# jiahuei/COMIC-Compact-Image-Captioning-with-Attention

Hardware: AMD Instinct MI355X
Metric: images/sec (decoder-mode XE training, COMIC-256, InceptionV3 frozen) (higher is better)
Workload: dtype bf16

## Files before the change

### comic-compact-image-captioning-with-attention_amd/_lib.py

```python
import ctypes as C
import os

_HERE = os.path.dirname(os.path.abspath(__file__))
LIB_PATH = os.environ.get('COMIC_HIP_LIB') or os.path.join(_HERE, 'lib', 'libcomic_hip.so')

c_void_p, c_int, c_int32, c_int64, c_float, c_double, c_char_p, c_uint64 = (
    C.c_void_p, C.c_int, C.c_int32, C.c_int64, C.c_float, C.c_double, C.c_char_p, C.c_uint64)


class CnnOp(C.Structure):
    _fields_ = [(n, c_int32) for n in (
        'kind', 'src', 'dst', 'src_coff', 'dst_coff', 'H', 'W', 'Cin', 'Cout', 'KH', 'KW', 'SH', 'SW',
        'PT', 'PL', 'Ho', 'Wo', 'weight', 'relu', 'out_f32', 'src_f32', 'lane', 'tile', 'group', 'flags', 'min_lds')]


class ImageDesc(C.Structure):
    _fields_ = [('offset', C.c_int64), ('in_h', c_int32), ('in_w', c_int32), ('flip', c_int32), ('oy', c_int32),
                ('ox', c_int32), ('sy', C.c_float), ('sx', C.c_float)]


class ConvWeight(C.Structure):
    _fields_ = [('w', c_void_p), ('scale', c_void_p), ('shift', c_void_p), ('w_frag', c_void_p)]


# ... 23 lines not shown
_DEC_ENV = (('COMIC_PERSIST', '0', DEC_NO_PERSIST), ('COMIC_PERSIST_BWD', '0', DEC_NO_PERSIST_BWD),
            ('COMIC_FUSED_STEP', '0', DEC_NO_FUSED_STEP), ('COMIC_SPLIT_ATTN_BWD', '0', DEC_NO_SPLIT_ATTN_BWD),
            ('COMIC_GRAD_LANES', '0', DEC_ONE_LANE), ('COMIC_SPLIT3', '0', DEC_EXACT_GEMM),
            ('COMIC_PERSIST_STAMPS', '1', DEC_STAMPS), ('COMIC_BEAM_LOGITS', '0', DEC_NO_BEAM_LOGITS),
            ('COMIC_LSTM_STREAM', '0', DEC_NO_LSTM_STREAM), ('COMIC_GROUP_GEMM', '0', DEC_NO_GROUP_GEMM),
            ('COMIC_BWD_OWN_ROWS', '1', DEC_BWD_OWN_ROWS))


def decoder_flags_from_env():
    f = 0
    for name, val, bit in _DEC_ENV:
        if os.environ.get(name, '')[:1] == val:
            f |= bit
    return f


CONV_TILES = 61
WS_TILE = 54
IMG_TILE = 55
CHAIN_TILE = 62
OP_RAW, OP_POOLED_SRC, OP_X3 = 1, 2, 4
OP_CHAIN_LINK = 8
OP_CHAIN_KEEP = 16
IM2COL_CONV_TILES = 12


def is_im2col_tile(tile):
    return tile <= IM2COL_CONV_TILES or 26 <= tile <= 47
PARAM_NAMES = ('W_init', 'K', 'b', 'W_m', 'W_v', 'W_q', 'v', 'ln_g', 'ln_b', 'tau', 'W_a', 'W_o', 'b_o', 'emb', 'cell_ln', 'K_c', 'b_c', 'status')


class DecoderParams(C.Structure):
    _fields_ = [(n, c_void_p) for n in PARAM_NAMES]


class BeamConstraints(C.Structure):
    _fields_ = [(n, c_int32) for n in ('min_length', 'no_repeat_ngram', 'ngram_stride', 'n_suppress')] + [
        ('suppress', c_int32 * 32)]


class GemmProb(C.Structure):
    _fields_ = [(n, c_void_p) for n in ('A', 'B', 'C', 'bias', 'mask')] + [(n, c_int32) for n in (
        'M', 'N', 'K', 'lda', 'ldb', 'ldc', 'ld_mask')] + [(n, c_float) for n in ('alpha', 'beta', 'keep')] + [
        ('type', c_int32), ('ones_a', c_int32)]


# ... 200 lines not shown
```

### comic-compact-image-captioning-with-attention_amd/csrc/conv.hip

```cpp
#include "conv_common.h"
#include "conv_ws.h"
#include "conv_stem.h"
#include "conv_img.h"
#include <cstdlib>
#include <cstring>
#include <algorithm>
#include <vector>

namespace {

constexpr int kRowBytes = 80;

template <typename T, int BM, int BN, int WM, int WN, bool MASK = false>
__global__ __launch_bounds__(256) void conv_igemm_kernel(ConvArgs a) {
  constexpr int EPC = Elem<T>::EPC;
  constexpr int BKE = 4 * EPC;
  constexpr int A_PASSES = (BM + 63) / 64;
  constexpr int B_PASSES = (BN + 63) / 64;
  constexpr int TM = BM / WM / 16;
  constexpr int TN = BN / WN / 16;
  static_assert(WM * WN == 4, "4 waves");

  __shared__ __attribute__((aligned(16))) unsigned char smem[2 * (BM + BN) * kRowBytes];
  unsigned char* Xs = smem;
// ... 2198 lines not shown
  while (j < n_ops && ops[j].group == ops[i].group) ++j;
  return j - i;
}

}

extern "C" long comic_cnn_group_args_bytes(const comic_cnn_op* ops, int n_ops) {
  long n = 0;
  for (int i = 0; i < n_ops; ++i) n += ops[i].group > 0;
  return n * (long)sizeof(ConvArgs);
}

extern "C" int comic_cnn_build_group_args(const comic_cnn_op* ops, int n_ops, void* const* buffers,
                                          const int32_t* buf_channels, const comic_conv_weight* weights, int batch,
                                          void* host_out) {
  COMIC_REQUIRE(ops && buffers && buf_channels && weights && host_out, "comic_cnn_build_group_args: null argument");
  ConvArgs* out = (ConvArgs*)host_out;
  for (int i = 0; i < n_ops;) {
    const int n = group_run(ops, n_ops, i);
    if (ops[i].group <= 0) {
      ++i;
      continue;
    }
    if (ws_group_selected(ops + i, n, batch)) {
      memset(out, 0, sizeof(ConvArgs) * n);
      out += n;
      i += n;
      continue;
    }
    COMIC_REQUIRE(ops[i].tile != COMIC_WS_TILE, "conv: group is not eligible for the weight-stationary 1x1 kernel");
    const int tile = group_tile(ops + i, n, batch);
    for (int j = 0; j < n; ++j)
      COMIC_REQUIRE(tile == COMIC_CHAIN_TILE || !(ops[i + j].flags & COMIC_OP_CHAIN_LINK),
                    "conv: COMIC_OP_CHAIN_LINK ops depend on each other -- their group runs on COMIC_CHAIN_TILE only (got tile %d)", tile);
    if (tile == COMIC_IMG_TILE || tile == COMIC_CHAIN_TILE) {
      memset(out, 0, sizeof(ConvArgs) * n);
      out += n;
      i += n;
      continue;
    }
    int blk = 0;
    for (int j = 0; j < n; ++j) {
      const comic_cnn_op* op = ops + i + j;
      const comic_conv_weight* wt = weights + op->weight;
      if (int rc = validate_grouped_conv(op, buf_channels[op->src], buf_channels[op->dst], wt, batch)) return rc;
      COMIC_REQUIRE(buffers[op->src] && buffers[op->dst], "grouped conv: null buffer");
      ConvArgs& a = out[j];
// ... 55 lines not shown
}

namespace {
struct Lanes {
  hipStream_t s[3];
  hipEvent_t fork_ev, join_ev[3];
  bool ok = false;
};
Lanes* get_lanes() {
  static Lanes lanes[16];
  int dev = 0;
  if (hipGetDevice(&dev) != hipSuccess || dev < 0 || dev >= 16) return nullptr;
  Lanes& l = lanes[dev];
  if (!l.ok) {
    for (int i = 0; i < 3; ++i) {
      if (hipStreamCreateWithFlags(&l.s[i], hipStreamNonBlocking) != hipSuccess) return nullptr;
      if (hipEventCreateWithFlags(&l.join_ev[i], hipEventDisableTiming) != hipSuccess) return nullptr;
    }
    if (hipEventCreateWithFlags(&l.fork_ev, hipEventDisableTiming) != hipSuccess) return nullptr;
    l.ok = true;
  }
  return &l;
}
}

template <typename HT>
static int cnn_forward_impl(const comic_cnn_op* ops, int n_ops, void* const* buffers, const int32_t* buf_channels,
                            const comic_conv_weight* weights, int batch, int dtype, const void* group_args_dev,
                            void* stream) {
  COMIC_REQUIRE(ops && buffers && buf_channels, "comic_cnn_forward: null table");
  const ConvArgs* gargs = (const ConvArgs*)group_args_dev;
  hipStream_t main_st = (hipStream_t)stream;
  Lanes* lanes = nullptr;
  bool used[3] = {false, false, false};
  for (int i = 0; i < n_ops; ++i) {
    const comic_cnn_op* op = ops + i;
    if (op->kind == 5) {
      if (!lanes) lanes = get_lanes();
      COMIC_REQUIRE(lanes, "comic_cnn_forward: cannot create branch streams");
      COMIC_REQUIRE(hipEventRecord(lanes->fork_ev, main_st) == hipSuccess, "fork: event record failed");
      for (int l = 0; l < 3; ++l) {
        COMIC_REQUIRE(hipStreamWaitEvent(lanes->s[l], lanes->fork_ev, 0) == hipSuccess, "fork: wait failed");
        used[l] = false;
      }
      continue;
    }
    if (op->kind == 6) {
      COMIC_REQUIRE(lanes, "join without fork");
      for (int l = 0; l < 3; ++l) {
        if (!used[l]) continue;
        COMIC_REQUIRE(hipEventRecord(lanes->join_ev[l], lanes->s[l]) == hipSuccess, "join: event record failed");
        COMIC_REQUIRE(hipStreamWaitEvent(main_st, lanes->join_ev[l], 0) == hipSuccess, "join: wait failed");
      }
      continue;
    }
    if (gargs && op->group > 0) {
      COMIC_REQUIRE(dtype == Half16<HT>::code && (op->kind == 0 || op->kind == 7) && op->lane == 0,
                    "grouped launch needs a bf16 or f16 plan and conv / pool+bn ops on the caller's stream");
      const int n = group_run(ops, n_ops, i);
      if (ws_group_selected(op, n, batch)) {
        if (int rc = run_ws_group<HT>(op, n, buffers, buf_channels, weights, batch, main_st)) return rc;
        gargs += n;
        i += n - 1;
        continue;
      }
      COMIC_REQUIRE(op->tile != COMIC_WS_TILE, "conv: group is not eligible for the weight-stationary 1x1 kernel");
      const int tile = group_tile(op, n, batch);
      for (int j = 0; j < n; ++j)
        COMIC_REQUIRE(tile == COMIC_CHAIN_TILE || !(op[j].flags & COMIC_OP_CHAIN_LINK),
                      "conv: COMIC_OP_CHAIN_LINK ops depend on each other -- their group runs on COMIC_CHAIN_TILE only (got tile %d)", tile);
      if (tile == COMIC_CHAIN_TILE) {
        if (int rc = launch_img_chains<HT>(op, n, buffers, buf_channels, weights, batch, main_st)) return rc;
        COMIC_LAUNCH_CHECK("image-resident conv chains");
        gargs += n;
        i += n - 1;
        continue;
      }
      if (tile == COMIC_IMG_TILE) {
// ... 32 lines not shown
        int lds = 0;
        const long nb = member_blocks(tile, a, &lds);
        COMIC_REQUIRE(nb >= 0, "grouped launch: member %d is not eligible for patch tile %d", j, tile);
        blocks += nb;
        lds_max = std::max(lds_max, lds);
      }
      COMIC_REQUIRE(blocks > 0 && blocks < (1L << 31), "grouped launch: bad workgroup count");
      if (is_walk_tile(tile)) blocks = (long)cdiv(batch * op->Ho * op->Wo, tile_bm(tile)) * walk_split(tile);
      if (!is_im2col_tile(tile)) {
        if (int rc = launch_patch_grouped_tile<HT>(tile, gargs, n, (int)blocks, std::max(lds_max, op->min_lds), main_st)) return rc;
      } else if (int rc = launch_dma_grouped_tile<HT>(tile, gargs, n, (int)blocks, op->min_lds, main_st)) {
        return rc;
      }
      COMIC_LAUNCH_CHECK("grouped conv");
      gargs += n;
      i += n - 1;
      continue;
    }
    hipStream_t st = main_st;
    if (op->lane > 0) {
      COMIC_REQUIRE(lanes && op->lane <= 3, "branch lane %d outside a fork/join region", op->lane);
      st = lanes->s[op->lane - 1];
      used[op->lane - 1] = true;
    }
    if (op->kind == 8 || op->kind == 9) {
      const bool with_1a = op->kind == 9;
      const int H0 = with_1a ? (op->H - 3) / 2 + 1 : op->H, W0 = with_1a ? (op->W - 3) / 2 + 1 : op->W;
      COMIC_REQUIRE(dtype == Half16<HT>::code && op->lane == 0, "stem stream: bf16 / f16 plans on the caller's stream only");
      COMIC_REQUIRE(op->Cin == (with_1a ? 3 : 32) && op->Cout == 64 && op->KH == 3 && op->KW == 3 && op->SH == 1 && op->SW == 1,
                    "stem stream: expects the (3 ->) 32 -> 32 -> 64 3x3 stem (got Cin %d, Cout %d)", op->Cin, op->Cout);
      COMIC_REQUIRE(comic_stem_stream_supported(H0, W0) && (!with_1a || comic_stem_stream_1a_supported(op->H, op->W)),
                    "stem stream: map %dx%d is not supported", op->H, op->W);
      const int Hp = (H0 - 2 - 3) / 2 + 1, Wp = (W0 - 2 - 3) / 2 + 1;
      COMIC_REQUIRE(op->Ho == Hp && op->Wo == Wp, "stem stream: Ho/Wo must be the pooled grid %dx%d", Hp, Wp);
      const comic_conv_weight* w0 = with_1a ? weights + op->weight : nullptr;
      const comic_conv_weight* wa = weights + op->weight + (with_1a ? 1 : 0);
      const comic_conv_weight* wb = wa + 1;
      const int xc = buf_channels[op->src], yc = buf_channels[op->dst];
      COMIC_REQUIRE(buffers[op->src] && buffers[op->dst] && wa->w && wb->w && wa->scale && wa->shift && wb->scale && wb->shift,
                    "stem stream: null buffer / weights");
      COMIC_REQUIRE(op->dst_coff + 64 <= yc && yc % 4 == 0 && op->dst_coff % 4 == 0, "stem stream: bad destination slice");
      COMIC_REQUIRE((long)batch * Hp * Wp * yc * 2 < (1L << 31), "stem stream: tensor too large");
      ComicStemArgs sa{};
      if (with_1a) {
        COMIC_REQUIRE(w0->w && w0->scale && w0->shift && xc == 3 && op->src_coff == 0, "stem stream: Conv2d_1a needs the whole fp32 image");
        sa.img = (const float*)buffers[op->src]; sa.Hi = op->H; sa.Wi = op->W;
        sa.w0 = (const float*)w0->w; sa.sc0 = w0->scale; sa.sh0 = w0->shift;
        sa.x = nullptr; sa.x_cs = 32; sa.x_co = 0;
      } else {
        COMIC_REQUIRE(op->src_coff + 32 <= xc && xc % 8 == 0 && op->src_coff % 8 == 0, "stem stream: bad source slice");
        COMIC_REQUIRE((long)batch * op->H * op->W * xc * 2 < (1L << 31), "stem stream: tensor too large");
        sa.x = (const bf16_t*)buffers[op->src]; sa.x_cs = xc; sa.x_co = op->src_coff;
      }
      sa.B = batch; sa.H0 = H0; sa.W0 = W0;
      sa.w1 = (const bf16_t*)wa->w; sa.w2 = (const bf16_t*)wb->w; sa.Kpad = (9 * 32 + 63) / 64 * 64;
      sa.sc1 = wa->scale; sa.sh1 = wa->shift; sa.sc2 = wb->scale; sa.sh2 = wb->shift;
      sa.y = (bf16_t*)buffers[op->dst]; sa.y_cs = yc; sa.y_co = op->dst_coff; sa.Hp = Hp; sa.Wp = Wp;
      sa.n_tasks = 2 * batch;
      sa.f16 = std::is_same<HT, f16_t>::value;
      if (int rc = comic_stem_stream_launch(sa, main_st)) return rc;
      COMIC_LAUNCH_CHECK("stem stream");
      continue;
    }
    const comic_conv_weight* wt = (op->kind <= 1 || op->kind == 7) ? weights + op->weight : nullptr;
    int rc = comic_conv2d_bn_relu(op, buffers[op->src], buf_channels[op->src], buffers[op->dst],
                                  buf_channels[op->dst], wt, batch, dtype, (void*)st);
    if (rc) return rc;
  }
  return 0;
}

extern "C" int comic_cnn_forward(const comic_cnn_op* ops, int n_ops, void* const* buffers, const int32_t* buf_channels,
                                 const comic_conv_weight* weights, int batch, int dtype, void* stream) {
  if (dtype == COMIC_F16) return cnn_forward_impl<f16_t>(ops, n_ops, buffers, buf_channels, weights, batch, dtype, nullptr, stream);
  return cnn_forward_impl<bf16_t>(ops, n_ops, buffers, buf_channels, weights, batch, dtype, nullptr, stream);
}

extern "C" int comic_cnn_forward_grouped(const comic_cnn_op* ops, int n_ops, void* const* buffers,
                                         const int32_t* buf_channels, const comic_conv_weight* weights, int batch,
                                         int dtype, const void* group_args_dev, void* stream) {
  COMIC_REQUIRE(group_args_dev || comic_cnn_group_args_bytes(ops, n_ops) == 0,
                "comic_cnn_forward_grouped: plan has grouped ops but no argument records");
  if (dtype == COMIC_F16)
    return cnn_forward_impl<f16_t>(ops, n_ops, buffers, buf_channels, weights, batch, dtype, group_args_dev, stream);
  return cnn_forward_impl<bf16_t>(ops, n_ops, buffers, buf_channels, weights, batch, dtype, group_args_dev, stream);
// ... 1484 lines not shown
```

### comic-compact-image-captioning-with-attention_amd/csrc/conv_stem.h

```cpp
#pragma once
#include "conv_common.h"

struct ComicStemArgs {
  const bf16_t* x;
  int B, H0, W0, x_cs, x_co;
  const bf16_t* w1;
  const bf16_t* w2;
  int Kpad;
  const float *sc1, *sh1, *sc2, *sh2;
  bf16_t* y;
  int y_cs, y_co, Hp, Wp;
  int n_tasks, parts;
  const float* img;
  int Hi, Wi;
  const float* w0;
  const float *sc0, *sh0;
  int f16;
};

bool comic_stem_stream_supported(int H0, int W0);
bool comic_stem_stream_1a_supported(int Hi, int Wi);
int comic_stem_stream_launch(const ComicStemArgs& a, hipStream_t st);
```

### comic-compact-image-captioning-with-attention_amd/csrc/conv_stem.hip

```cpp
#include <algorithm>

#include "conv_common.h"
#include "conv_stem.h"

namespace {

constexpr int kPxB = 96;
constexpr int kRowPx = 132;
constexpr int kRowB = kRowPx * kPxB;
constexpr int kRing = 4;
constexpr int kTableFloats = 2 * (32 + 64);
constexpr int kImgRing = 16;

#define STEM_BARRIER()                                    \
  do {                                                    \
    asm volatile("s_waitcnt lgkmcnt(0)" ::: "memory");    \
    __builtin_amdgcn_s_barrier();                         \
    asm volatile("" ::: "memory");                        \
  } while (0)

__device__ __forceinline__ float row_next1(float v) { return dpp_move<0x12F>(v, v); }
__device__ __forceinline__ float row_next2(float v) { return dpp_move<0x12E>(v, v); }

template <typename HT, bool FUSE1A>
__global__ __launch_bounds__(512) void conv_stem_stream_kernel(ComicStemArgs a) {
  extern __shared__ __attribute__((aligned(16))) unsigned char smem[];
  float* table = (float*)smem;
  unsigned char* xring = smem + kTableFloats * 4;
  unsigned char* yring = xring + kRing * kRowB;
  float* imgring = (float*)(yring + kRing * kRowB);

  const int tid = threadIdx.x, lane = tid & 63;
  const int wave = __builtin_amdgcn_readfirstlane(tid >> 6);
  const int H1 = a.H0 - 2, W1 = a.W0 - 2;
  const int part_rows = (a.Hp + a.parts - 1) / a.parts;

  if (tid < 32) {
    table[tid] = a.sc1[tid];
    table[32 + tid] = a.sh1[tid];
  }
  if (tid < 64) {
    table[64 + tid] = a.sc2[tid];
    table[128 + tid] = a.sh2[tid];
  }
  for (int i = tid; i < kRing * kRowPx * (kPxB / 16); i += 512) *(uint4*)(yring + i * 16) = make_uint4(0, 0, 0, 0);
  if constexpr (FUSE1A)
    for (int i = tid; i < kImgRing * a.Wi * 3 / 4; i += 512) *(float4*)(imgring + 4 * i) = make_float4(0.f, 0.f, 0.f, 0.f);

  const int fr = lane & 15, fg = lane >> 4;
  const uint32_t x_lane = (uint32_t)(fr * kPxB + fg * 16);

  if (wave >= 4) {
    const int wv = wave - 4;
    const int p = wv & 1, hh = wv >> 1;
    const int y1_start = 64 * hh;
    const bool y1_work = y1_start < W1;
    const int ltid = tid - 256;
    int px[2], ch[2];
    bool act[2];
#pragma unroll
    for (int i = 0; i < 2; ++i) {
      const int c = ltid + 256 * i;
      px[i] = c >> 2;
      ch[i] = c & 3;
      act[i] = px[i] < a.W0;
    }
    uint32_t goff[2];
#pragma unroll
// ... 82 lines not shown
        const int x = 32 * wv + 16 * i + fr;
        const int x6 = 6 * min(x, a.W0 - 1);
        float xv[8];
#pragma unroll
        for (int s8 = 0; s8 < 8; ++s8) xv[s8] = imgring[rb[s8] + x6];
        uint32_t hh[4], ll[4];
#pragma unroll
        for (int e = 0; e < 4; ++e) {
          hh[e] = pack_bf16x2(xv[2 * e], xv[2 * e + 1]);
          ll[e] = pack_bf16x2(xv[2 * e] - __uint_as_float(hh[e] << 16), xv[2 * e + 1] - __uint_as_float(hh[e] & 0xFFFF0000u));
        }
        const bf16x8_t xh = __builtin_bit_cast(bf16x8_t, make_uint4(hh[0], hh[1], hh[2], hh[3]));
        const bf16x8_t xl = __builtin_bit_cast(bf16x8_t, make_uint4(ll[0], ll[1], ll[2], ll[3]));
#pragma unroll
        for (int n = 0; n < 2; ++n) {
          f32x4_t acc0 = (f32x4_t){0.f, 0.f, 0.f, 0.f};
          acc0 = __builtin_amdgcn_mfma_f32_16x16x32_bf16(w0h[n], xh, acc0, 0, 0, 0);
          acc0 = __builtin_amdgcn_mfma_f32_16x16x32_bf16(w0h[n], xl, acc0, 0, 0, 0);
          acc0 = __builtin_amdgcn_mfma_f32_16x16x32_bf16(w0l[n], xh, acc0, 0, 0, 0);
          const float v0 = fmaxf(fmaf(acc0[0], sc0[n].x, sh0[n].x), 0.f), v1 = fmaxf(fmaf(acc0[1], sc0[n].y, sh0[n].y), 0.f);
          const float v2 = fmaxf(fmaf(acc0[2], sc0[n].z, sh0[n].z), 0.f), v3 = fmaxf(fmaf(acc0[3], sc0[n].w, sh0[n].w), 0.f);
          if (x < a.W0) *(uint2*)(dst + x * kPxB + n * 32) = make_uint2(Half16<HT>::pack(v0, v1), Half16<HT>::pack(v2, v3));
        }
      }
    };
    STEM_BARRIER();
    const float4 sc1 = *(const float4*)(table + p * 16 + fg * 4), sh1 = *(const float4*)(table + 32 + p * 16 + fg * 4);
    for (int task = blockIdx.x; task < a.n_tasks; task += gridDim.x) {
      const int b = task / a.parts, h = task - b * a.parts;
      const int p0 = h * part_rows, p1 = min(a.Hp, p0 + part_rows) - 1;
      const int qa = 2 * p0 - 1, r_last = 2 * p1 + 2;
      const int nsteps = r_last + 2 - qa + 1;
      Row r0, r1, r2;
      ImgRows ia, ib, ic;
      if constexpr (FUSE1A) {
        const int ir0 = 2 * max(qa, 0), ir1 = min(2 * (qa + 3) + 2, a.Hi - 1);
        const float4* src = (const float4*)(a.img + ((size_t)b * a.Hi + ir0) * rowf);
        for (int i = ltid; i < (ir1 - ir0 + 1) * row4; i += 256) {
          const int r = ir0 + i / row4, c4 = i % row4;
          *(float4*)(imgring + (size_t)(r & (kImgRing - 1)) * rowf + 4 * c4) = src[i];
        }
        ia = load_img(b, qa + 4);
        ib = load_img(b, qa + 5);
        STEM_BARRIER();
        compute_x0(qa);
        compute_x0(qa + 1);
// ... 37 lines not shown
            }
            __builtin_amdgcn_s_setprio(0);
          }
          unsigned char* dst = yring + ((q + 8) & 3) * kRowB + (p * 16 + fg * 4) * 2;
#pragma unroll
          for (int j = 0; j < 4; ++j) {
            const int x = y1_start + j * 16 + fr;
            float v0 = fmaxf(fmaf(acc[j][0], sc1.x, sh1.x), 0.f), v1 = fmaxf(fmaf(acc[j][1], sc1.y, sh1.y), 0.f);
            float v2 = fmaxf(fmaf(acc[j][2], sc1.z, sh1.z), 0.f), v3 = fmaxf(fmaf(acc[j][3], sc1.w, sh1.w), 0.f);
            if (!real) v0 = v1 = v2 = v3 = 0.f;
            if (x < W1) *(uint2*)(dst + (x + 1) * kPxB) = make_uint2(Half16<HT>::pack(v0, v1), Half16<HT>::pack(v2, v3));
          }
        }
        if constexpr (FUSE1A) {
          compute_x0(q + 3);
          store_img(q + 4, ia);
          ia = ib;
          ib = ic;
        } else {
          store_row(q + 3, r0);
          r0 = r1;
          r1 = r2;
        }
        STEM_BARRIER();
      }
    }
    return;
  }

  const int p = wave & 1, hh = wave >> 1;
  const int y2_start = 56 * hh;
  const bool y2_work = y2_start < W1;
  constexpr int kTileStep = 14;
  bf16x8_t w2[2][9];
#pragma unroll
  for (int i = 0; i < 2; ++i) {
    const bf16_t* wp2 = a.w2 + (size_t)((2 * p + i) * 16 + fr) * a.Kpad + fg * 8;
#pragma unroll
    for (int tap = 0; tap < 9; ++tap) w2[i][tap] = __builtin_bit_cast(bf16x8_t, *(const uint4*)(wp2 + tap * 32));
  }
  STEM_BARRIER();
  float4 sc2[2], sh2[2];
#pragma unroll
  for (int i = 0; i < 2; ++i) {
    sc2[i] = *(const float4*)(table + 64 + (2 * p + i) * 16 + fg * 4);
    sh2[i] = *(const float4*)(table + 128 + (2 * p + i) * 16 + fg * 4);
  }

// ... 48 lines not shown
      const int prow = p0 + (rel >> 1) - 1;
#pragma unroll
      for (int i = 0; i < 2; ++i) {
        f32x4_t v[4];
#pragma unroll
        for (int j = 0; j < 4; ++j)
#pragma unroll
          for (int e = 0; e < 4; ++e) {
            v[j][e] = fmaxf(run[i][j][e], acc[i][j][e]);
            run[i][j][e] = acc[i][j][e];
          }
#pragma unroll
        for (int j = 0; j < 4; ++j) {
          float o[4];
#pragma unroll
          for (int e = 0; e < 4; ++e)
            o[e] = fmaxf(fmaxf(v[j][e], row_next1(v[j][e])), row_next2(v[j][e]));
          const float o0 = fmaxf(fmaf(o[0], sc2[i].x, sh2[i].x), 0.f), o1 = fmaxf(fmaf(o[1], sc2[i].y, sh2[i].y), 0.f);
          const float o2 = fmaxf(fmaf(o[2], sc2[i].z, sh2[i].z), 0.f), o3 = fmaxf(fmaf(o[3], sc2[i].w, sh2[i].w), 0.f);
          const int x = y2_start + j * kTileStep + fr;
          const int jc = x >> 1;
          if ((fr & 1) == 0 && fr <= 12 && jc < a.Wp) {
            bf16_t* yp = a.y + ((size_t)((b * a.Hp + prow) * a.Wp + jc)) * a.y_cs + a.y_co + (2 * p + i) * 16 + fg * 4;
            *(uint2*)yp = make_uint2(Half16<HT>::pack(o0, o1), Half16<HT>::pack(o2, o3));
          }
        }
      }
    };
    f32x4_t acc[2][4];
    for (int t = 0; t < nsteps; ++t) {
      const int r = qa + t - 2;
      if (y2_work && r >= r_first && r <= r_last) {
        mfma_row(r, acc);
        pool_row(r, acc);
      }
      STEM_BARRIER();
    }
  }
}

}

bool comic_stem_stream_supported(int H0, int W0) {
  const int Wp = (W0 - 2 - 3) / 2 + 1;
  return H0 >= 7 && W0 >= 7 && Wp <= 56;
}

bool comic_stem_stream_1a_supported(int Hi, int Wi) {
  const int H0 = (Hi - 3) / 2 + 1, W0 = (Wi - 3) / 2 + 1;
  return Hi >= 17 && Wi % 4 == 0 && 2 * (Wi * 3 / 4) <= 512 && comic_stem_stream_supported(H0, W0) &&
         kTableFloats * 4 + 2 * kRing * kRowB + kImgRing * Wi * 3 * 4 <= 160 * 1024;
}

namespace {
template <typename HT>
int stem_stream_launch(const ComicStemArgs& a_in, hipStream_t st) {
  ComicStemArgs a = a_in;
  if (!comic_stem_stream_supported(a.H0, a.W0) || (a.img && !comic_stem_stream_1a_supported(a.Hi, a.Wi))) {
    comic_set_error("conv_stem: unsupported map %dx%d", a.H0, a.W0);
    return 2;
  }
  const int lds = kTableFloats * 4 + 2 * kRing * kRowB + (a.img ? kImgRing * a.Wi * 3 * 4 : 0);
  static PerDeviceOnce attr_once__;
  bool& attr_set = attr_once__.slot();
  if (!attr_set) {
    if (hipFuncSetAttribute((const void*)conv_stem_stream_kernel<HT, false>, hipFuncAttributeMaxDynamicSharedMemorySize,
                            160 * 1024) != hipSuccess ||
        hipFuncSetAttribute((const void*)conv_stem_stream_kernel<HT, true>, hipFuncAttributeMaxDynamicSharedMemorySize,
                            160 * 1024) != hipSuccess) {
      comic_set_error("conv_stem: cannot reserve %d bytes of LDS", lds);
      return 1;
    }
    attr_set = true;
  }
  int dev = 0, cus = 256;
  if (hipGetDevice(&dev) == hipSuccess) (void)hipDeviceGetAttribute(&cus, hipDeviceAttributeMultiprocessorCount, dev);
  a.parts = 2;
  while (a.parts < 8 && a.B * a.parts < cus && (a.Hp + 2 * a.parts - 1) / (2 * a.parts) >= 6) a.parts *= 2;
  a.n_tasks = a.B * a.parts;
  const int grid = std::min(a.n_tasks, cus);
  if (a.img)
    hipLaunchKernelGGL((conv_stem_stream_kernel<HT, true>), dim3(grid), dim3(512), lds, st, a);
  else
    hipLaunchKernelGGL((conv_stem_stream_kernel<HT, false>), dim3(grid), dim3(512), lds, st, a);
  return 0;
}
}

int comic_stem_stream_launch(const ComicStemArgs& a, hipStream_t st) {
  return a.f16 ? stem_stream_launch<f16_t>(a, st) : stem_stream_launch<bf16_t>(a, st);
}
```

### comic-compact-image-captioning-with-attention_amd/nets.py

```python
from __future__ import annotations

import ctypes as C
import json
import math
import os

import numpy as np

from . import _lib as L
from . import streams

BN_EPS = 1e-3

_STEM = [('c', 'Conv2d_1a_3x3', 32, (3, 3), 2, 'VALID'), ('c', 'Conv2d_2a_3x3', 32, (3, 3), 1, 'VALID'),
         ('c', 'Conv2d_2b_3x3', 64, (3, 3), 1, 'SAME'), ('max', 'MaxPool_3a_3x3'),
         ('c', 'Conv2d_3b_1x1', 80, (1, 1), 1, 'VALID'), ('c', 'Conv2d_4a_3x3', 192, (3, 3), 1, 'VALID'),
         ('max', 'MaxPool_5a_3x3')]


def _c(scope, cout, k, stride=1, pad='SAME'):
    return ('c', scope, cout, k if isinstance(k, tuple) else (k, k), stride, pad)


def _mixed5(pool_c, b1):
# ... 59 lines not shown

def stem_stream_supported(H0, W0):
    return H0 >= 7 and W0 >= 7 and (W0 - 2 - 3) // 2 + 1 <= 56


def stem_stream_1a_supported(Hi, Wi):
    H0, W0 = (Hi - 3) // 2 + 1, (Wi - 3) // 2 + 1
    return (Hi >= 17 and Wi % 4 == 0 and 2 * (Wi * 3 // 4) <= 512 and stem_stream_supported(H0, W0)
            and 2 * (32 + 64) * 4 + 2 * 4 * 132 * 96 + 16 * Wi * 3 * 4 <= 160 * 1024)


def _out(size, k, s, pad):
    if pad == 'SAME':
        o = -(-size // s)
        tot = max((o - 1) * s + k - size, 0)
        return o, tot // 2
    return (size - k) // s + 1, 0


class CnnPlan:

    def __init__(self, name='inception_v3', image_size=(224, 224), final_endpoint='Mixed_7c', branch_streams=False,
                 group_branches=True, layers=None, pool_after_projection=False, ride_pools=False, side_pools=None,
                 fuse_pools=False, x3=False, fuse_stem_1a=True, fuse_chains=None):
        if name not in ('inception_v3', 'inception_v1', 'chain'):
            raise NotImplementedError('only inception_v3 / inception_v1 are on the MI355X hot path (got %r)' % name)
        self.name = name
        self.ops = []
        self.buffers = []
        self.weights = []
        self.wphys = []
        self.fm_src = None
        self.end_points = {}
        self.macs = 0
        self._lane = 0
        self._branch = None
        self.branch_streams = branch_streams
        self.group_branches = group_branches and not branch_streams
        self._depth = 0
        self._next_group = 1
        self.pool_after_projection = pool_after_projection
        self.ride_pools = ride_pools
        self.side_pools = bool(side_pools)
        self.fuse_pools = bool(fuse_pools)
        self.fuse_stem_1a = bool(fuse_stem_1a)
        bf16_grouped = not x3 and self.group_branches and name == 'inception_v3' and not self.ride_pools
        self.fuse_chains = bf16_grouped if fuse_chains is None else bool(fuse_chains)
        self.keep_chain_maps = not self.pool_after_projection
        self.small_batch_plan = None
        if fuse_chains is None and self.fuse_chains:
            self.small_batch_plan = CnnPlan(name, image_size, final_endpoint, branch_streams, group_branches, layers,
                                            pool_after_projection, ride_pools, side_pools, fuse_pools, x3, fuse_stem_1a,
                                            fuse_chains=False)
        if self.fuse_chains and (x3 or not self.group_branches):
            raise ValueError('fuse_chains needs a grouped bf16 plan')
        if self.fuse_pools and not (pool_after_projection and name == 'inception_v3'):
            raise ValueError('fuse_pools needs an inception_v3 plan with pool_after_projection=True')
        self._pooled_src = None
        self._logical = {}
        self.block_ranges = []
        if name == 'chain':
            self._build_chain(image_size, layers)
        elif name == 'inception_v1':
            self._build_v1(image_size, 'Mixed_4f' if final_endpoint == 'Mixed_7c' else final_endpoint)
        else:
            self._build_v3(image_size, final_endpoint)
        self.x3 = bool(x3)
        if self.x3:
            if fuse_pools or self._logical or name == 'inception_v1':
                raise ValueError('x3 plans: InceptionV3 / chain layouts only (no folded max-pools, no padded channels)')
            for o in self.ops:
                if o['kind'] == 0:
                    o['Cin'] *= 3
                if o['kind'] in (0, 1, 2, 3, 7):
                    o['flags'] = o.get('flags', 0) | L.OP_X3
            self.buffers = [(H, W, Cc if f32 else 3 * Cc, f32) for (H, W, Cc, f32) in self.buffers]
# ... 254 lines not shown
            self.end_points[bname] = cur
        if fm_endpoint not in self.end_points:
            raise ValueError('unknown feature-map end point %r' % fm_endpoint)
        self._finish_head(cur)
        if fm_endpoint != 'Mixed_5c':
            self.fm_src = self.end_points[fm_endpoint]
            self.fm = None

    def _build_v3(self, image_size, final_endpoint):
        H, W = image_size
        cur = self._buf(H, W, 3, True)
        self.input = cur
        root = 'InceptionV3'
        stem = list(_STEM)
        if self.fuse_pools and stem_stream_supported(*self._stem_dims(H, W)):
            if self.fuse_stem_1a and stem_stream_1a_supported(H, W):
                cur = self._stem_stream(cur, root, stem[1], stem[2], spec_1a=stem[0])
            else:
                cur, _ = self._conv(cur, root, stem[0])
                self.end_points[stem[0][1]] = cur
                cur = self._stem_stream(cur, root, stem[1], stem[2])
            self.end_points[stem[3][1]] = cur
            stem = stem[4:]
        for op in stem:
            if op[0] == 'c':
                cur, _ = self._conv(cur, root, op)
                self._pooled_src = None
            elif self.fuse_pools:
                Hc, Wc = self.buffers[cur][:2]
                self._pooled_src = (cur, _out(Hc, 3, 2, 'VALID')[0], _out(Wc, 3, 2, 'VALID')[0])
                continue
            else:
                cur, _ = self._pool(cur, 2, 3, 2, 'VALID')
            self.end_points[op[1]] = cur
        self.block_ranges.append([0, len(self.ops)])
        for bname, branches in INCEPTION_V3_BLOCKS:
            Hi, Wi, Ci, _ = self.buffers[cur]
            block_first = len(self.ops)
            if self._pooled_src is not None:
                assert self._pooled_src[0] == cur and all(b[0][0] == 'c' and b[0][3] == (1, 1) or b[0][0] == 'avg'
                                                          for b in branches)
                Hi, Wi = self._pooled_src[1:]
            outs = [self._branch_out(b, Hi, Wi, Ci) for b in branches]
            Ho, Wo = outs[0][0], outs[0][1]
            Ctot = sum(o[2] for o in outs)
            last = bname == final_endpoint
            blk = self._buf(Ho, Wo, Ctot, f32=last)
            coff = 0
            if self.branch_streams:
                self.ops.append(self._sync_op(5))
            first_op = len(self.ops)
            for bi, branch in enumerate(branches):
                scope = '%s/%s/Branch_%d' % (root, bname, bi)
                self._lane = bi if self.branch_streams else 0
                self._branch = bi
                x = cur
                if (self.pool_after_projection and len(branch) == 2 and branch[0][0] == 'avg' and branch[1][0] == 'c'
                        and branch[1][3] == (1, 1) and branch[1][2] % 16 == 0):
# ... 604 lines not shown
    def _drop_graphs(self):
        self._graph, self._calls = None, 0
        for a in self._alt.values():
            a[1], a[2] = None, 0

    def _run(self, bufptr=None):
        bufptr = bufptr or self._bufptr
        if self._group_args is not None:
            L.check(self.lib.comic_cnn_forward_grouped(self._ops, len(self.plan.ops), bufptr, self._bufch,
                                                       self._wt, self.batch, self.dcode,
                                                       self._group_args.data_ptr(), L.stream_ptr()),
                    'cnn_forward_grouped')
            return
        L.check(self.lib.comic_cnn_forward(self._ops, len(self.plan.ops), bufptr, self._bufch, self._wt,
                                           self.batch, self.dcode, L.stream_ptr()), 'cnn_forward')

    def _adopt(self, images):
        key = images.data_ptr()
        a = self._alt.get(key)
        if a is not None:
            return a
        if len(self._alt) >= 4 or not images.is_contiguous() or self._train is not None:
            return None
        if any(o['src'] == self.plan.input and o.get('group', 0) for o in self.plan.ops):
            return None
        bp = (C.c_void_p * len(self.bufs))(*[b.data_ptr() for b in self.bufs])
        bp[self.plan.input] = key
        a = self._alt[key] = [bp, None, 0, images]
        return a

    def forward(self, images, use_graph=False):
        inp = self.bufs[self.plan.input]
        assert images.shape == inp.shape and images.dtype == inp.dtype, (images.shape, inp.shape)
        alt = None
        if images.data_ptr() != inp.data_ptr():
            alt = self._adopt(images)
            if alt is None:
                inp.copy_(images)
        bufptr, graph, calls = (alt[0], alt[1], alt[2]) if alt is not None else (None, self._graph, self._calls)
        self._last_bufptr = bufptr
        if use_graph and graph is None and calls >= 1:
            graph = self.torch.cuda.CUDAGraph()
            with self.torch.cuda.graph(graph, capture_error_mode='thread_local'):
                self._run(bufptr)
            if alt is not None:
                alt[1] = graph
            else:
# ... 39 lines not shown
                    self._ops[i].tile = int(t)
                if self._group_args is not None:
                    self._build_group_args()
                self._drop_graphs()
                return {i: (None, t) for i, t in enumerate(tiles)}
        chosen = self._autotune(reps, verbose, torch, st)
        if cache:
            store_tune_cache(cache, self._tune_key(), [int(self._ops[i].tile) for i in range(len(self.plan.ops))])
        return chosen

    def _autotune(self, reps, verbose, torch, st):
        chosen = {}
        ev0, ev1 = torch.cuda.Event(enable_timing=True), torch.cuda.Event(enable_timing=True)
        n_ops = len(self.plan.ops)
        grouped = self._group_args is not None
        rec_bytes = 0
        if grouped:
            n_rec = sum(1 for j in range(n_ops) if self._ops[j].group > 0)
            rec_bytes = self.lib.comic_cnn_group_args_bytes(self._ops, n_ops) // n_rec
        rec = 0
        i = 0
        while i < n_ops:
            o = self.plan.ops[i]
            if o['kind'] != 0:
                i += 1
                continue
            op = self._ops[i]
            if o.get('flags', 0) & L.OP_POOLED_SRC or o.get('tile') == L.CHAIN_TILE:
                n = 1
                while i + n < n_ops and op.group > 0 and self._ops[i + n].group == op.group:
                    n += 1
                rec += n if (grouped and op.group > 0) else 0
                i += n
                continue
            n = 1
            if grouped and op.group > 0:
                while i + n < n_ops and self._ops[i + n].group == op.group:
                    n += 1
                first = C.byref(self._ops, i * C.sizeof(L.CnnOp))
                rec_off = rec * rec_bytes

                def run():
                    L.check(self.lib.comic_cnn_forward_grouped(first, n, self._bufptr, self._bufch, self._wt,
                                                               self.batch, self.dcode,
                                                               self._group_args.data_ptr() + rec_off, st),
                            'grouped conv (autotune)')
                rec += n
            else:
                src, dst = self.bufs[o['src']], self.bufs[o['dst']]
                wt = self._wt[o['weight']]
# ... 76 lines not shown
```

### include/comic_hip.h

```cpp
#ifndef COMIC_HIP_H_
#define COMIC_HIP_H_

#include <stddef.h>
#include <stdint.h>

#ifdef __cplusplus
extern "C" {
#endif

#define COMIC_F32 0
#define COMIC_BF16 1
#define COMIC_F16 2
#define COMIC_ABI_VERSION 1
#define COMIC_CONV_TILES 61
#define COMIC_WS_TILE 54
#define COMIC_IMG_TILE 55
#define COMIC_CHAIN_TILE 62

const char* comic_last_error(void);
int comic_abi_version(void);
int comic_device_count(void);


int comic_pack_conv_weights(const float* w_hwio, void* w_packed, int kh, int kw, int cin, int cout,
// ... 3 lines not shown
                  float* shift, int c, void* stream);

typedef struct comic_cnn_op {
  int32_t kind;
  int32_t src, dst;
  int32_t src_coff, dst_coff;
  int32_t H, W, Cin, Cout, KH, KW, SH, SW, PT, PL, Ho, Wo;
  int32_t weight;
  int32_t relu;
  int32_t out_f32;
  int32_t src_f32;
  int32_t lane;
  int32_t tile;
  int32_t group;
  int32_t flags;
  int32_t min_lds;
} comic_cnn_op;
#define COMIC_OP_RAW 1
#define COMIC_OP_POOLED_SRC 2

#define COMIC_OP_X3 4
#define COMIC_OP_CHAIN_LINK 8
#define COMIC_OP_CHAIN_KEEP 16

typedef struct comic_conv_weight {
  const void* w;
  const float* scale;
  const float* shift;
  const void* w_frag;
} comic_conv_weight;

int comic_cnn_forward(const comic_cnn_op* ops, int n_ops, void* const* buffers,
                      const int32_t* buf_channels, const comic_conv_weight* weights, int batch,
                      int dtype, void* stream);

int comic_cnn_pack_frag_weights(const void* w_plan, void* w_frag, const int64_t* table_dev, int n_weights,
                                int64_t total_elems, void* stream);

long comic_cnn_group_args_bytes(const comic_cnn_op* ops, int n_ops);
int comic_cnn_build_group_args(const comic_cnn_op* ops, int n_ops, void* const* buffers,
                               const int32_t* buf_channels, const comic_conv_weight* weights,
                               int batch, void* host_out);
int comic_cnn_forward_grouped(const comic_cnn_op* ops, int n_ops, void* const* buffers,
                              const int32_t* buf_channels, const comic_conv_weight* weights,
                              int batch, int dtype, const void* group_args_dev, void* stream);

// ... 284 lines not shown
```

Measured before the change: 39640.

## Fuse the Conv2d_3b 1x1 conv into the stem stream kernel

New measurement: 39700 (median of 2 runs). About the same (+0.1%).

```diff
diff --git a/comic-compact-image-captioning-with-attention_amd/_lib.py b/comic-compact-image-captioning-with-attention_amd/_lib.py
--- a/comic-compact-image-captioning-with-attention_amd/_lib.py
+++ b/comic-compact-image-captioning-with-attention_amd/_lib.py
@@ -69,6 +69,7 @@
 OP_RAW, OP_POOLED_SRC, OP_X3 = 1, 2, 4
 OP_CHAIN_LINK = 8
 OP_CHAIN_KEEP = 16
+OP_CARRIED = 32
 IM2COL_CONV_TILES = 12
 
 
diff --git a/comic-compact-image-captioning-with-attention_amd/csrc/conv.hip b/comic-compact-image-captioning-with-attention_amd/csrc/conv.hip
--- a/comic-compact-image-captioning-with-attention_amd/csrc/conv.hip
+++ b/comic-compact-image-captioning-with-attention_amd/csrc/conv.hip
@@ -2244,7 +2244,7 @@
       ++i;
       continue;
     }
-    if (ws_group_selected(ops + i, n, batch)) {
+    if (ops[i].kind == 8 || ops[i].kind == 9 || ws_group_selected(ops + i, n, batch)) {
       memset(out, 0, sizeof(ConvArgs) * n);
       out += n;
       i += n;
@@ -2346,6 +2346,70 @@
   }
   return &l;
 }
+}
+
+template <typename HT>
+static int run_stem_stream(const comic_cnn_op* ops, int n_ops, int i, const comic_cnn_op* carried, void* const* buffers,
+                           const int32_t* buf_channels, const comic_conv_weight* weights, int batch, int dtype, hipStream_t st) {
+  const comic_cnn_op* op = ops + i;
+  const bool with_1a = op->kind == 9;
+  const int H0 = with_1a ? (op->H - 3) / 2 + 1 : op->H, W0 = with_1a ? (op->W - 3) / 2 + 1 : op->W;
+  COMIC_REQUIRE(dtype == Half16<HT>::code && op->lane == 0, "stem stream: bf16 / f16 plans on the caller's stream only");
+  COMIC_REQUIRE(op->Cin == (with_1a ? 3 : 32) && op->Cout == 64 && op->KH == 3 && op->KW == 3 && op->SH == 1 && op->SW == 1,
+                "stem stream: expects the (3 ->) 32 -> 32 -> 64 3x3 stem (got Cin %d, Cout %d)", op->Cin, op->Cout);
+  COMIC_REQUIRE(comic_stem_stream_supported(H0, W0) && (!with_1a || comic_stem_stream_1a_supported(op->H, op->W)),
+                "stem stream: map %dx%d is not supported", op->H, op->W);
+  const int Hp = (H0 - 2 - 3) / 2 + 1, Wp = (W0 - 2 - 3) / 2 + 1;
+  COMIC_REQUIRE(op->Ho == Hp && op->Wo == Wp, "stem stream: Ho/Wo must be the pooled grid %dx%d", Hp, Wp);
+  const comic_conv_weight* w0 = with_1a ? weights + op->weight : nullptr;
+  const comic_conv_weight* wa = weights + op->weight + (with_1a ? 1 : 0);
+  const comic_conv_weight* wb = wa + 1;
+  const int xc = buf_channels[op->src], yc = buf_channels[op->dst];
+  COMIC_REQUIRE(buffers[op->src] && buffers[op->dst] && wa->w && wb->w && wa->scale && wa->shift && wb->scale && wb->shift,
+                "stem stream: null buffer / weights");
+  COMIC_REQUIRE(op->dst_coff + 64 <= yc && yc % 4 == 0 && op->dst_coff % 4 == 0, "stem stream: bad destination slice");
+  COMIC_REQUIRE((long)batch * Hp * Wp * yc * 2 < (1L << 31), "stem stream: tensor too large");
+  ComicStemArgs sa{};
+  if (with_1a) {
+    COMIC_REQUIRE(w0->w && w0->scale && w0->shift && xc == 3 && op->src_coff == 0, "stem stream: Conv2d_1a needs the whole fp32 image");
+    sa.img = (const float*)buffers[op->src]; sa.Hi = op->H; sa.Wi = op->W;
+    sa.w0 = (const float*)w0->w; sa.sc0 = w0->scale; sa.sh0 = w0->shift;
+    sa.x = nullptr; sa.x_cs = 32; sa.x_co = 0;
+  } else {
+    COMIC_REQUIRE(op->src_coff + 32 <= xc && xc % 8 == 0 && op->src_coff % 8 == 0, "stem stream: bad source slice");
+    COMIC_REQUIRE((long)batch * op->H * op->W * xc * 2 < (1L << 31), "stem stream: tensor too large");
+    sa.x = (const bf16_t*)buffers[op->src]; sa.x_cs = xc; sa.x_co = op->src_coff;
+  }
+  sa.B = batch; sa.H0 = H0; sa.W0 = W0;
+  sa.w1 = (const bf16_t*)wa->w; sa.w2 = (const bf16_t*)wb->w; sa.Kpad = (9 * 32 + 63) / 64 * 64;
+  sa.sc1 = wa->scale; sa.sh1 = wa->shift; sa.sc2 = wb->scale; sa.sh2 = wb->shift;
+  sa.y = (bf16_t*)buffers[op->dst]; sa.y_cs = yc; sa.y_co = op->dst_coff; sa.Hp = Hp; sa.Wp = Wp;
+  sa.n_tasks = 2 * batch;
+  sa.f16 = std::is_same<HT, f16_t>::value;
+  if (carried) {
+    const comic_cnn_op& c = *carried;
+    const comic_conv_weight* w3 = weights + c.weight;
+    COMIC_REQUIRE(c.kind == 0 && c.group == op->group && op->group > 0 && c.lane == 0,
+                  "stem stream: the carried conv shares the stream's group id");
+    COMIC_REQUIRE(c.KH == 1 && c.KW == 1 && c.SH == 1 && c.SW == 1 && c.PT == 0 && c.PL == 0 && c.Cin == 64 && c.Cout >= 16 &&
+                  c.Cout <= 80 && c.Cout % 16 == 0 && c.relu && !c.out_f32 && !(c.flags & ~COMIC_OP_CARRIED),
+                  "stem stream: carries a plain 1x1 conv 64 -> 16..80 channels (a multiple of 16) + BN + ReLU (got %dx%d, %d -> %d, flags %d)",
+                  c.KH, c.KW, c.Cin, c.Cout, c.flags);
+    COMIC_REQUIRE(c.src == op->dst && c.src_coff == op->dst_coff && c.H == Hp && c.W == Wp && c.Ho == Hp && c.Wo == Wp,
+                  "stem stream: the carried conv reads the whole pooled map");
+    for (int j = 0; j < n_ops; ++j)
+      COMIC_REQUIRE(j == i || ops + j == carried || ops[j].kind == 5 || ops[j].kind == 6 || ops[j].src != op->dst,
+                    "stem stream: the carried conv must be the pooled map's only reader (op %d reads it too)", j);
+    const int y3c = buf_channels[c.dst];
+    COMIC_REQUIRE(buffers[c.dst] && w3->w && w3->scale && w3->shift, "stem stream: carried conv: null buffer / weights");
+    COMIC_REQUIRE(c.dst_coff + c.Cout <= y3c && y3c % 4 == 0 && c.dst_coff % 4 == 0, "stem stream: carried conv: bad destination slice");
+    COMIC_REQUIRE((long)batch * Hp * Wp * y3c * 2 < (1L << 31), "stem stream: tensor too large");
+    sa.w3 = (const bf16_t*)w3->w; sa.sc3 = w3->scale; sa.sh3 = w3->shift;
+    sa.y3 = (bf16_t*)buffers[c.dst]; sa.y3_cs = y3c; sa.y3_co = c.dst_coff; sa.C3 = c.Cout;
+  }
+  if (int rc = comic_stem_stream_launch(sa, st)) return rc;
+  COMIC_LAUNCH_CHECK("stem stream");
+  return 0;
 }
 
 template <typename HT>
@@ -2378,6 +2442,15 @@
       }
       continue;
     }
+    if (op->kind == 8 || op->kind == 9) {
+      const comic_cnn_op* carried = (i + 1 < n_ops && (ops[i + 1].flags & COMIC_OP_CARRIED)) ? ops + i + 1 : nullptr;
+      if (int rc = run_stem_stream<HT>(ops, n_ops, i, carried, buffers, buf_channels, weights, batch, dtype, main_st)) return rc;
+      const int n = carried ? 2 : 1;
+      if (gargs && op->group > 0) gargs += n;
+      i += n - 1;
+      continue;
+    }
+    COMIC_REQUIRE(!(op->flags & COMIC_OP_CARRIED), "conv: a COMIC_OP_CARRIED conv must follow the stem stream op that carries it");
     if (gargs && op->group > 0) {
       COMIC_REQUIRE(dtype == Half16<HT>::code && (op->kind == 0 || op->kind == 7) && op->lane == 0,
                     "grouped launch needs a bf16 or f16 plan and conv / pool+bn ops on the caller's stream");
@@ -2456,45 +2529,6 @@
       COMIC_REQUIRE(lanes && op->lane <= 3, "branch lane %d outside a fork/join region", op->lane);
       st = lanes->s[op->lane - 1];
       used[op->lane - 1] = true;
-    }
-    if (op->kind == 8 || op->kind == 9) {
-      const bool with_1a = op->kind == 9;
-      const int H0 = with_1a ? (op->H - 3) / 2 + 1 : op->H, W0 = with_1a ? (op->W - 3) / 2 + 1 : op->W;
-      COMIC_REQUIRE(dtype == Half16<HT>::code && op->lane == 0, "stem stream: bf16 / f16 plans on the caller's stream only");
-      COMIC_REQUIRE(op->Cin == (with_1a ? 3 : 32) && op->Cout == 64 && op->KH == 3 && op->KW == 3 && op->SH == 1 && op->SW == 1,
-                    "stem stream: expects the (3 ->) 32 -> 32 -> 64 3x3 stem (got Cin %d, Cout %d)", op->Cin, op->Cout);
-      COMIC_REQUIRE(comic_stem_stream_supported(H0, W0) && (!with_1a || comic_stem_stream_1a_supported(op->H, op->W)),
-                    "stem stream: map %dx%d is not supported", op->H, op->W);
-      const int Hp = (H0 - 2 - 3) / 2 + 1, Wp = (W0 - 2 - 3) / 2 + 1;
-      COMIC_REQUIRE(op->Ho == Hp && op->Wo == Wp, "stem stream: Ho/Wo must be the pooled grid %dx%d", Hp, Wp);
-      const comic_conv_weight* w0 = with_1a ? weights + op->weight : nullptr;
-      const comic_conv_weight* wa = weights + op->weight + (with_1a ? 1 : 0);
-      const comic_conv_weight* wb = wa + 1;
-      const int xc = buf_channels[op->src], yc = buf_channels[op->dst];
-      COMIC_REQUIRE(buffers[op->src] && buffers[op->dst] && wa->w && wb->w && wa->scale && wa->shift && wb->scale && wb->shift,
-                    "stem stream: null buffer / weights");
-      COMIC_REQUIRE(op->dst_coff + 64 <= yc && yc % 4 == 0 && op->dst_coff % 4 == 0, "stem stream: bad destination slice");
-      COMIC_REQUIRE((long)batch * Hp * Wp * yc * 2 < (1L << 31), "stem stream: tensor too large");
-      ComicStemArgs sa{};
-      if (with_1a) {
-        COMIC_REQUIRE(w0->w && w0->scale && w0->shift && xc == 3 && op->src_coff == 0, "stem stream: Conv2d_1a needs the whole fp32 image");
-        sa.img = (const float*)buffers[op->src]; sa.Hi = op->H; sa.Wi = op->W;
-        sa.w0 = (const float*)w0->w; sa.sc0 = w0->scale; sa.sh0 = w0->shift;
-        sa.x = nullptr; sa.x_cs = 32; sa.x_co = 0;
-      } else {
-        COMIC_REQUIRE(op->src_coff + 32 <= xc && xc % 8 == 0 && op->src_coff % 8 == 0, "stem stream: bad source slice");
-        COMIC_REQUIRE((long)batch * op->H * op->W * xc * 2 < (1L << 31), "stem stream: tensor too large");
-        sa.x = (const bf16_t*)buffers[op->src]; sa.x_cs = xc; sa.x_co = op->src_coff;
-      }
-      sa.B = batch; sa.H0 = H0; sa.W0 = W0;
-      sa.w1 = (const bf16_t*)wa->w; sa.w2 = (const bf16_t*)wb->w; sa.Kpad = (9 * 32 + 63) / 64 * 64;
-      sa.sc1 = wa->scale; sa.sh1 = wa->shift; sa.sc2 = wb->scale; sa.sh2 = wb->shift;
-      sa.y = (bf16_t*)buffers[op->dst]; sa.y_cs = yc; sa.y_co = op->dst_coff; sa.Hp = Hp; sa.Wp = Wp;
-      sa.n_tasks = 2 * batch;
-      sa.f16 = std::is_same<HT, f16_t>::value;
-      if (int rc = comic_stem_stream_launch(sa, main_st)) return rc;
-      COMIC_LAUNCH_CHECK("stem stream");
-      continue;
     }
     const comic_conv_weight* wt = (op->kind <= 1 || op->kind == 7) ? weights + op->weight : nullptr;
     int rc = comic_conv2d_bn_relu(op, buffers[op->src], buf_channels[op->src], buffers[op->dst],
diff --git a/comic-compact-image-captioning-with-attention_amd/csrc/conv_stem.h b/comic-compact-image-captioning-with-attention_amd/csrc/conv_stem.h
--- a/comic-compact-image-captioning-with-attention_amd/csrc/conv_stem.h
+++ b/comic-compact-image-captioning-with-attention_amd/csrc/conv_stem.h
@@ -15,6 +15,10 @@
   int Hi, Wi;
   const float* w0;
   const float *sc0, *sh0;
+  const bf16_t* w3;
+  const float *sc3, *sh3;
+  bf16_t* y3;
+  int y3_cs, y3_co, C3;
   int f16;
 };
 
diff --git a/comic-compact-image-captioning-with-attention_amd/csrc/conv_stem.hip b/comic-compact-image-captioning-with-attention_amd/csrc/conv_stem.hip
--- a/comic-compact-image-captioning-with-attention_amd/csrc/conv_stem.hip
+++ b/comic-compact-image-captioning-with-attention_amd/csrc/conv_stem.hip
@@ -11,6 +11,10 @@
 constexpr int kRing = 4;
 constexpr int kTableFloats = 2 * (32 + 64);
 constexpr int kImgRing = 16;
+constexpr int kPoolPxB = 160;
+constexpr int kPoolPx = 64;
+constexpr int kC3 = 80;
+constexpr int k3bBytes = kPoolPx * kPoolPxB + 2 * kC3 * 4;
 
 #define STEM_BARRIER()                                    \
   do {                                                    \
@@ -22,13 +26,15 @@
 __device__ __forceinline__ float row_next1(float v) { return dpp_move<0x12F>(v, v); }
 __device__ __forceinline__ float row_next2(float v) { return dpp_move<0x12E>(v, v); }
 
-template <typename HT, bool FUSE1A>
+template <typename HT, bool FUSE1A, bool FUSE3B>
 __global__ __launch_bounds__(512) void conv_stem_stream_kernel(ComicStemArgs a) {
   extern __shared__ __attribute__((aligned(16))) unsigned char smem[];
   float* table = (float*)smem;
   unsigned char* xring = smem + kTableFloats * 4;
   unsigned char* yring = xring + kRing * kRowB;
   float* imgring = (float*)(yring + kRing * kRowB);
+  unsigned char* poolrow = (unsigned char*)imgring + (FUSE1A ? kImgRing * a.Wi * 3 * 4 : 0);
+  float* table3 = (float*)(poolrow + kPoolPx * kPoolPxB);
 
   const int tid = threadIdx.x, lane = tid & 63;
   const int wave = __builtin_amdgcn_readfirstlane(tid >> 6);
@@ -44,6 +50,13 @@
     table[128 + tid] = a.sh2[tid];
   }
   for (int i = tid; i < kRing * kRowPx * (kPxB / 16); i += 512) *(uint4*)(yring + i * 16) = make_uint4(0, 0, 0, 0);
+  if constexpr (FUSE3B) {
+    for (int i = tid; i < kPoolPx * kPoolPxB / 16; i += 512) *(uint4*)(poolrow + i * 16) = make_uint4(0, 0, 0, 0);
+    if (tid < kC3) {
+      table3[tid] = tid < a.C3 ? a.sc3[tid] : 0.f;
+      table3[kC3 + tid] = tid < a.C3 ? a.sh3[tid] : 0.f;
+    }
+  }
   if constexpr (FUSE1A)
     for (int i = tid; i < kImgRing * a.Wi * 3 / 4; i += 512) *(float4*)(imgring + 4 * i) = make_float4(0.f, 0.f, 0.f, 0.f);
 
@@ -172,6 +185,35 @@
           const float v2 = fmaxf(fmaf(acc0[2], sc0[n].z, sh0[n].z), 0.f), v3 = fmaxf(fmaf(acc0[3], sc0[n].w, sh0[n].w), 0.f);
           if (x < a.W0) *(uint2*)(dst + x * kPxB + n * 32) = make_uint2(Half16<HT>::pack(v0, v1), Half16<HT>::pack(v2, v3));
         }
+      }
+    };
+    bf16x8_t w3[kC3 / 16][2];
+    if constexpr (FUSE3B) {
+#pragma unroll
+      for (int n = 0; n < kC3 / 16; ++n)
+#pragma unroll
+        for (int ks = 0; ks < 2; ++ks) {
+          uint4 v = make_uint4(0, 0, 0, 0);
+          if (n * 16 < a.C3) v = *(const uint4*)(a.w3 + (size_t)(n * 16 + fr) * 64 + ks * 32 + fg * 8);
+          w3[n][ks] = __builtin_bit_cast(bf16x8_t, v);
+        }
+    }
+    auto conv3b_row = [&](int b, int prow) {
+      const int x = 16 * wv + fr;
+      if (!(16 * wv < a.Wp)) return;
+      const unsigned char* src = poolrow + x * kPoolPxB + fg * 16;
+      const bf16x8_t x0 = __builtin_bit_cast(bf16x8_t, *(const uint4*)src);
+      const bf16x8_t x1 = __builtin_bit_cast(bf16x8_t, *(const uint4*)(src + 64));
+      bf16_t* yp = a.y3 + ((size_t)((b * a.Hp + prow) * a.Wp + min(x, a.Wp - 1))) * a.y3_cs + a.y3_co + fg * 4;
+#pragma unroll
+      for (int n = 0; n < kC3 / 16; ++n) {
+        f32x4_t acc3 = (f32x4_t){0.f, 0.f, 0.f, 0.f};
+        acc3 = Half16<HT>::mfma(w3[n][0], x0, acc3);
+        acc3 = Half16<HT>::mfma(w3[n][1], x1, acc3);
+        const float4 sc = *(const float4*)(table3 + n * 16 + fg * 4), sh = *(const float4*)(table3 + kC3 + n * 16 + fg * 4);
+        const float v0 = fmaxf(fmaf(acc3[0], sc.x, sh.x), 0.f), v1 = fmaxf(fmaf(acc3[1], sc.y, sh.y), 0.f);
+        const float v2 = fmaxf(fmaf(acc3[2], sc.z, sh.z), 0.f), v3 = fmaxf(fmaf(acc3[3], sc.w, sh.w), 0.f);
+        if (x < a.Wp && n * 16 < a.C3) *(uint2*)(yp + n * 16) = make_uint2(Half16<HT>::pack(v0, v1), Half16<HT>::pack(v2, v3));
       }
     };
     STEM_BARRIER();
@@ -255,8 +297,11 @@
           r0 = r1;
           r1 = r2;
         }
+        if constexpr (FUSE3B)
+          if (t >= 6 && (t & 1) == 0) conv3b_row(b, p0 + ((t - 4) >> 1) - 1);
         STEM_BARRIER();
       }
+      if constexpr (FUSE3B) conv3b_row(b, p1);
     }
     return;
   }
@@ -351,7 +396,9 @@
           const int jc = x >> 1;
           if ((fr & 1) == 0 && fr <= 12 && jc < a.Wp) {
             bf16_t* yp = a.y + ((size_t)((b * a.Hp + prow) * a.Wp + jc)) * a.y_cs + a.y_co + (2 * p + i) * 16 + fg * 4;
-            *(uint2*)yp = make_uint2(Half16<HT>::pack(o0, o1), Half16<HT>::pack(o2, o3));
+            const uint2 o16 = make_uint2(Half16<HT>::pack(o0, o1), Half16<HT>::pack(o2, o3));
+            *(uint2*)yp = o16;
+            if constexpr (FUSE3B) *(uint2*)(poolrow + jc * kPoolPxB + ((2 * p + i) * 16 + fg * 4) * 2) = o16;
           }
         }
       }
@@ -389,14 +436,21 @@
     comic_set_error("conv_stem: unsupported map %dx%d", a.H0, a.W0);
     return 2;
   }
-  const int lds = kTableFloats * 4 + 2 * kRing * kRowB + (a.img ? kImgRing * a.Wi * 3 * 4 : 0);
+  const bool with_3b = a.w3 != nullptr;
+  const int lds = kTableFloats * 4 + 2 * kRing * kRowB + (a.img ? kImgRing * a.Wi * 3 * 4 : 0) + (with_3b ? k3bBytes : 0);
+  if (with_3b && (a.C3 < 16 || a.C3 > kC3 || a.C3 % 16 != 0 || !a.sc3 || !a.sh3 || !a.y3 || lds > 160 * 1024)) {
+    comic_set_error("conv_stem: the carried 1x1 conv needs 64 -> 16..80 channels (a multiple of 16) and %d bytes of LDS (got %d channels)",
+                    lds, a.C3);
+    return 2;
+  }
   static PerDeviceOnce attr_once__;
   bool& attr_set = attr_once__.slot();
   if (!attr_set) {
-    if (hipFuncSetAttribute((const void*)conv_stem_stream_kernel<HT, false>, hipFuncAttributeMaxDynamicSharedMemorySize,
-                            160 * 1024) != hipSuccess ||
-        hipFuncSetAttribute((const void*)conv_stem_stream_kernel<HT, true>, hipFuncAttributeMaxDynamicSharedMemorySize,
-                            160 * 1024) != hipSuccess) {
+    const void* kernels[4] = {(const void*)conv_stem_stream_kernel<HT, false, false>, (const void*)conv_stem_stream_kernel<HT, true, false>,
+                              (const void*)conv_stem_stream_kernel<HT, false, true>, (const void*)conv_stem_stream_kernel<HT, true, true>};
+    bool ok = true;
+    for (const void* k : kernels) ok = ok && hipFuncSetAttribute(k, hipFuncAttributeMaxDynamicSharedMemorySize, 160 * 1024) == hipSuccess;
+    if (!ok) {
       comic_set_error("conv_stem: cannot reserve %d bytes of LDS", lds);
       return 1;
     }
@@ -408,10 +462,14 @@
   while (a.parts < 8 && a.B * a.parts < cus && (a.Hp + 2 * a.parts - 1) / (2 * a.parts) >= 6) a.parts *= 2;
   a.n_tasks = a.B * a.parts;
   const int grid = std::min(a.n_tasks, cus);
-  if (a.img)
-    hipLaunchKernelGGL((conv_stem_stream_kernel<HT, true>), dim3(grid), dim3(512), lds, st, a);
+  if (a.img && with_3b)
+    hipLaunchKernelGGL((conv_stem_stream_kernel<HT, true, true>), dim3(grid), dim3(512), lds, st, a);
+  else if (a.img)
+    hipLaunchKernelGGL((conv_stem_stream_kernel<HT, true, false>), dim3(grid), dim3(512), lds, st, a);
+  else if (with_3b)
+    hipLaunchKernelGGL((conv_stem_stream_kernel<HT, false, true>), dim3(grid), dim3(512), lds, st, a);
   else
-    hipLaunchKernelGGL((conv_stem_stream_kernel<HT, false>), dim3(grid), dim3(512), lds, st, a);
+    hipLaunchKernelGGL((conv_stem_stream_kernel<HT, false, false>), dim3(grid), dim3(512), lds, st, a);
   return 0;
 }
 }
diff --git a/comic-compact-image-captioning-with-attention_amd/nets.py b/comic-compact-image-captioning-with-attention_amd/nets.py
--- a/comic-compact-image-captioning-with-attention_amd/nets.py
+++ b/comic-compact-image-captioning-with-attention_amd/nets.py
@@ -105,7 +105,7 @@
 
     def __init__(self, name='inception_v3', image_size=(224, 224), final_endpoint='Mixed_7c', branch_streams=False,
                  group_branches=True, layers=None, pool_after_projection=False, ride_pools=False, side_pools=None,
-                 fuse_pools=False, x3=False, fuse_stem_1a=True, fuse_chains=None):
+                 fuse_pools=False, x3=False, fuse_stem_1a=True, fuse_chains=None, fuse_stem_3b=True):
         if name not in ('inception_v3', 'inception_v1', 'chain'):
             raise NotImplementedError('only inception_v3 / inception_v1 are on the MI355X hot path (got %r)' % name)
         self.name = name
@@ -127,6 +127,7 @@
         self.side_pools = bool(side_pools)
         self.fuse_pools = bool(fuse_pools)
         self.fuse_stem_1a = bool(fuse_stem_1a)
+        self.fuse_stem_3b = bool(fuse_stem_3b)
         bf16_grouped = not x3 and self.group_branches and name == 'inception_v3' and not self.ride_pools
         self.fuse_chains = bf16_grouped if fuse_chains is None else bool(fuse_chains)
         self.keep_chain_maps = not self.pool_after_projection
@@ -134,7 +135,7 @@
         if fuse_chains is None and self.fuse_chains:
             self.small_batch_plan = CnnPlan(name, image_size, final_endpoint, branch_streams, group_branches, layers,
                                             pool_after_projection, ride_pools, side_pools, fuse_pools, x3, fuse_stem_1a,
-                                            fuse_chains=False)
+                                            fuse_chains=False, fuse_stem_3b=fuse_stem_3b)
         if self.fuse_chains and (x3 or not self.group_branches):
             raise ValueError('fuse_chains needs a grouped bf16 plan')
         if self.fuse_pools and not (pool_after_projection and name == 'inception_v3'):
@@ -435,6 +436,14 @@
                 cur = self._stem_stream(cur, root, stem[1], stem[2])
             self.end_points[stem[3][1]] = cur
             stem = stem[4:]
+            if self.fuse_stem_3b and stem[0][0] == 'c' and stem[0][2:] == (80, (1, 1), 1, 'VALID'):
+                carrier = self.ops[-1]
+                cur, _ = self._conv(cur, root, stem[0])
+                self.end_points[stem[0][1]] = cur
+                carrier['group'] = self.ops[-1]['group'] = self._next_group
+                self._next_group += 1
+                self.ops[-1]['flags'] |= L.OP_CARRIED
+                stem = stem[1:]
         for op in stem:
             if op[0] == 'c':
                 cur, _ = self._conv(cur, root, op)
@@ -447,6 +456,11 @@
                 cur, _ = self._pool(cur, 2, 3, 2, 'VALID')
             self.end_points[op[1]] = cur
         self.block_ranges.append([0, len(self.ops)])
+        if final_endpoint in self.end_points:
+            self._pooled_src = None
+            self._finish_head(cur)
+            self.fm_src, self.fm = self.end_points[final_endpoint], None
+            return
         for bname, branches in INCEPTION_V3_BLOCKS:
             Hi, Wi, Ci, _ = self.buffers[cur]
             block_first = len(self.ops)
@@ -1097,7 +1111,7 @@
             return a
         if len(self._alt) >= 4 or not images.is_contiguous() or self._train is not None:
             return None
-        if any(o['src'] == self.plan.input and o.get('group', 0) for o in self.plan.ops):
+        if any(o['src'] == self.plan.input and o.get('group', 0) and o['kind'] not in (8, 9) for o in self.plan.ops):
             return None
         bp = (C.c_void_p * len(self.bufs))(*[b.data_ptr() for b in self.bufs])
         bp[self.plan.input] = key
@@ -1183,10 +1197,17 @@
         i = 0
         while i < n_ops:
             o = self.plan.ops[i]
+            op = self._ops[i]
+            if o['kind'] in (8, 9) and op.group > 0:
+                n = 1
+                while i + n < n_ops and self._ops[i + n].group == op.group:
+                    n += 1
+                rec += n if grouped else 0
+                i += n
+                continue
             if o['kind'] != 0:
                 i += 1
                 continue
-            op = self._ops[i]
             if o.get('flags', 0) & L.OP_POOLED_SRC or o.get('tile') == L.CHAIN_TILE:
                 n = 1
                 while i + n < n_ops and op.group > 0 and self._ops[i + n].group == op.group:
diff --git a/include/comic_hip.h b/include/comic_hip.h
--- a/include/comic_hip.h
+++ b/include/comic_hip.h
@@ -49,6 +49,7 @@
 #define COMIC_OP_X3 4
 #define COMIC_OP_CHAIN_LINK 8
 #define COMIC_OP_CHAIN_KEEP 16
+#define COMIC_OP_CARRIED 32
 
 typedef struct comic_conv_weight {
   const void* w;
```
